# agnusmaximus/Word2Bits

Measured on AMD Instinct MI355X. Metric: training words/sec at dim=800 bitlevel=1 neg=24, higher is better.
Workload: dtype f32

## Files before the change

### word2bits_amd/csrc/w2b_device.hpp

```cpp
#pragma once
#include "w2b_internal.h"
#include <type_traits>

#ifndef W2B_T
#define W2B_T 13
#endif
#ifndef W2B_T_LOSS
#define W2B_T_LOSS W2B_T
#endif
template <bool LOSS> struct TFor { static constexpr int value = LOSS ? W2B_T_LOSS : W2B_T; };
#ifndef W2B_CA
#define W2B_CA 8
#endif
#ifndef W2B_STASH
#define W2B_STASH 8
#endif
#ifndef W2B_MINWAVES
#define W2B_MINWAVES 4
#endif

namespace {

struct QParam { int bitlevel; int steps_i; float steps_f; };

template <int QM>
__device__ __forceinline__ float quant(float x, const QParam &q) {
  if (QM == 0) return x;
  if (QM == 2) {
    const float lvl = (__builtin_fabsf(x) <= .5f) ? .25f : .75f;
    return (x < 0.f) ? -lvl : lvl;
  }
  const float sgn = (x < 0.f) ? -1.f : 1.f;
  if (QM == 1) return sgn / 3.f;
  const float mag = x * sgn;
  float lvl = 0.f;
  if (q.bitlevel >= 4) {
    int k = (int)(mag * q.steps_f + .5f);
    k = k > q.steps_i ? q.steps_i : k;
    lvl = (float)k / q.steps_f;
  }
  return sgn * lvl;
}
__device__ __forceinline__ QParam make_qparam(const W2bParams &P) {
  QParam qp;
  qp.bitlevel = P.bitlevel;
  qp.steps_i = (P.bitlevel >= 4) ? (1 << (P.bitlevel - 1)) : 1;
  qp.steps_f = (float)qp.steps_i;
  return qp;
}

template <int VEC> struct Col { float e[VEC]; };

#define W2B_MM_EXACT 4
#define W2B_EXACT_COLS 256
#ifndef W2B_XCD_STORE_AUX
#define W2B_XCD_STORE_AUX 2
#endif
template <int MM> struct Aux {
  static constexpr int load = (MM == 0 || MM == W2B_MM_EXACT) ? 16 : ((MM == 2 || MM == 5 || MM == 6) ? 2 : 0);
  static constexpr int store = (MM == 1) ? 0 : ((MM == 5) ? 2 : ((MM == 6) ? W2B_XCD_STORE_AUX : 16));
};
typedef unsigned int u32x4 __attribute__((ext_vector_type(4)));
typedef unsigned int u32x2 __attribute__((ext_vector_type(2)));
template <int VEC, int MM, int TB = -1>
__device__ __forceinline__ Col<VEC> load_col(const float *tab, long long row, int dim, int col0, unsigned tab_bytes) {
  Col<VEC> c;
  const int urow = __builtin_amdgcn_readfirstlane((int)row);
  __amdgpu_buffer_rsrc_t r;
  int soff;
  if (TB == 0 || (TB < 0 && tab_bytes)) {
    r = __builtin_amdgcn_make_buffer_rsrc((void *)tab, 0, (int)tab_bytes, 0x27000);
    soff = urow * dim * 4;
  } else {
    r = __builtin_amdgcn_make_buffer_rsrc((void *)(tab + urow * (long long)dim), 0, dim * 4, 0x27000);
    soff = 0;
  }
  if (VEC == 4) {
    u32x4 t = __builtin_amdgcn_raw_buffer_load_b128(r, col0 * 4, soff, Aux<MM>::load);
    c.e[0] = __uint_as_float(t.x); c.e[1 % VEC] = __uint_as_float(t.y);
    c.e[2 % VEC] = __uint_as_float(t.z); c.e[3 % VEC] = __uint_as_float(t.w);
  } else if (VEC == 2) {
    u32x2 t = __builtin_amdgcn_raw_buffer_load_b64(r, col0 * 4, soff, Aux<MM>::load);
    c.e[0] = __uint_as_float(t.x); c.e[1 % VEC] = __uint_as_float(t.y);
  } else {
    c.e[0] = __uint_as_float(__builtin_amdgcn_raw_buffer_load_b32(r, col0 * 4, soff, Aux<MM>::load));
  }
  return c;
}
template <int VEC, int MM, int TB = -1>
__device__ __forceinline__ void store_col(float *tab, long long row, int dim, int col0, const Col<VEC> &c,
                                          unsigned tab_bytes) {
  const int urow = __builtin_amdgcn_readfirstlane((int)row);
  __amdgpu_buffer_rsrc_t r;
  int soff;
  if (TB == 0 || (TB < 0 && tab_bytes)) {
    r = __builtin_amdgcn_make_buffer_rsrc((void *)tab, 0, (int)tab_bytes, 0x27000);
    soff = urow * dim * 4;
  } else {
    r = __builtin_amdgcn_make_buffer_rsrc((void *)(tab + urow * (long long)dim), 0, dim * 4, 0x27000);
    soff = 0;
  }
  if (VEC == 4) {
    u32x4 t;
    t.x = __float_as_uint(c.e[0]); t.y = __float_as_uint(c.e[1 % VEC]);
    t.z = __float_as_uint(c.e[2 % VEC]); t.w = __float_as_uint(c.e[3 % VEC]);
    __builtin_amdgcn_raw_buffer_store_b128(t, r, col0 * 4, soff, Aux<MM>::store);
  } else if (VEC == 2) {
    u32x2 t;
    t.x = __float_as_uint(c.e[0]); t.y = __float_as_uint(c.e[1 % VEC]);
    __builtin_amdgcn_raw_buffer_store_b64(t, r, col0 * 4, soff, Aux<MM>::store);
  } else {
    __builtin_amdgcn_raw_buffer_store_b32(__float_as_uint(c.e[0]), r, col0 * 4, soff, Aux<MM>::store);
  }
}

template <int CTRL, int ROW_MASK>
__device__ __forceinline__ float dpp_f(float x) {
  return __int_as_float(__builtin_amdgcn_update_dpp(0, __float_as_int(x), CTRL, ROW_MASK, 0xf, false));
}
template <int CTRL, int ROW_MASK>
__device__ __forceinline__ unsigned dpp_u(unsigned x) {
  return (unsigned)__builtin_amdgcn_update_dpp(0, (int)x, CTRL, ROW_MASK, 0xf, false);
}
#define W2B_DPP_QUAD_1032 0xB1
#define W2B_DPP_QUAD_2301 0x4E
#define W2B_DPP_ROW_HALF_MIRROR 0x141
#define W2B_DPP_ROW_MIRROR 0x140
#define W2B_DPP_ROW_BCAST15 0x142
#define W2B_DPP_ROW_BCAST31 0x143
__device__ __forceinline__ float wave_sum(float x) {
  x += dpp_f<W2B_DPP_QUAD_1032, 0xf>(x);
  x += dpp_f<W2B_DPP_QUAD_2301, 0xf>(x);
  x += dpp_f<W2B_DPP_ROW_HALF_MIRROR, 0xf>(x);
  x += dpp_f<W2B_DPP_ROW_MIRROR, 0xf>(x);
  x += dpp_f<W2B_DPP_ROW_BCAST15, 0xa>(x);
  x += dpp_f<W2B_DPP_ROW_BCAST31, 0xc>(x);
  return __int_as_float(__builtin_amdgcn_readlane(__float_as_int(x), 63));
}
__device__ __forceinline__ unsigned wave_xor(unsigned x) {
  x ^= dpp_u<W2B_DPP_QUAD_1032, 0xf>(x);
  x ^= dpp_u<W2B_DPP_QUAD_2301, 0xf>(x);
  x ^= dpp_u<W2B_DPP_ROW_HALF_MIRROR, 0xf>(x);
  x ^= dpp_u<W2B_DPP_ROW_MIRROR, 0xf>(x);
  x ^= dpp_u<W2B_DPP_ROW_BCAST15, 0xa>(x);
  x ^= dpp_u<W2B_DPP_ROW_BCAST31, 0xc>(x);
  return (unsigned)__builtin_amdgcn_readlane((int)x, 63);
}
__device__ __forceinline__ double wave_sum_d(double x) {
#pragma unroll
  for (int o = 32; o > 0; o >>= 1) x += __shfl_xor(x, o, 64);
  return x;
}
#define W2B_WAVE_SYNC() do { __builtin_amdgcn_fence(__ATOMIC_RELEASE, "wavefront"); __builtin_amdgcn_wave_barrier(); __builtin_amdgcn_fence(__ATOMIC_ACQUIRE, "wavefront"); } while (0)
__device__ __forceinline__ unsigned long long lane_lt_mask(int lane) {
  return lane == 0 ? 0ull : (~0ull >> (64 - lane));
}

#define W2B_LDS __attribute__((address_space(3)))
typedef float f32x4_t __attribute__((ext_vector_type(4)));
__device__ __forceinline__ Col<4> lds_ld(const W2B_LDS float *p) {
  const f32x4_t t = *(const W2B_LDS f32x4_t *)p;
  Col<4> c;
  c.e[0] = t.x; c.e[1] = t.y; c.e[2] = t.z; c.e[3] = t.w;
  return c;
}
__device__ __forceinline__ void lds_st(W2B_LDS float *p, const Col<4> &c) {
  f32x4_t t;
  t.x = c.e[0]; t.y = c.e[1]; t.z = c.e[2]; t.w = c.e[3];
  *(W2B_LDS f32x4_t *)p = t;
}

#ifdef W2B_PHASE_TIMERS
#define W2B_TICK(k) do { if (timing_) { const unsigned long long n_ = __builtin_readcyclecounter(); \
    atomicAdd(&P.shared->dbg[k], n_ - tick_); tick_ = n_; } } while (0)
#define W2B_COUNT(k) do { if (timing_) atomicAdd(&P.shared->dbg[k], 1ull); } while (0)
#else
#define W2B_TICK(k) do { } while (0)
#define W2B_COUNT(k) do { } while (0)
#endif

struct WordLds {
  int *ctx;
  int *umult;
  int *tgt;
  int *prev;
  int *cend;
  float *red;
  float *stash;
  float *xprod;
};

__device__ __forceinline__ int round4(int x) { return (x + 3) & ~3; }

__device__ __forceinline__ WordLds carve_word_lds(int *base, int window, int negative, int vec) {
  const int maxc = round4(2 * window + 1), maxt = round4(negative + 1);
  WordLds L;
  L.stash = reinterpret_cast<float *>(base);
  base += W2B_STASH * blockDim.x * vec;
  L.red = reinterpret_cast<float *>(base);
  int *p = base + 2 * W2B_T * W2B_MAXW;
  L.ctx = p; p += maxc;
  L.umult = p; p += maxc;
  L.tgt = p; p += maxt;
  L.prev = p; p += maxt;
  L.cend = p; p += maxt;
  L.xprod = nullptr;
  return L;
}


template <int T, typename IP>
__device__ __forceinline__ int prep_lists(IP tgt, IP prev, IP cend, int nt, IP ctx, IP umult, int cw,
                                          int lane) {
  W2B_WAVE_SYNC();
  for (int i0 = 0; i0 < nt; i0 += 64) {
    const int i = i0 + lane;
    const int me = (i < nt) ? tgt[i] : -1;
    int pd = -1;
    for (int j = 0; j < min(nt, i0 + 64); j++) {
      const int tj = (j >= i0) ? __builtin_amdgcn_readlane(me, j - i0) : tgt[j];
      pd = (j < i && tj == me) ? j : pd;
    }
    if (i < nt) prev[i] = pd;
  }
  if (umult) {
    for (int i0 = 0; i0 < cw; i0 += 64) {
      const int i = i0 + lane;
      const int me = (i < cw) ? ctx[i] : -1;
      bool first = true;
      int mult = 0;
      for (int j = 0; j < cw; j++) {
        const int cj = (j >= i0 && j < i0 + 64) ? __builtin_amdgcn_readlane(me, j - i0) : ctx[j];
        first = first && !(j < i && cj == me);
        mult += (j >= i && cj == me) ? 1 : 0;
      }
      if (i < cw) umult[i] = first ? mult : 0;
    }
  }
  W2B_WAVE_SYNC();
  int start = 0, k = 0;
  while (start < nt) {
    const int lim = min(start + T, nt);
    int end = lim;
    for (int i0 = start + 1; i0 < lim; i0 += 64) {
      const int i = i0 + lane;
      const bool hit = (i < lim) && (prev[i] >= start);
      const unsigned long long m = __ballot(hit);
      if (m) { end = i0 + __ffsll((long long)m) - 1; break; }
    }
    if (lane == 0) cend[k] = end;
    k++;
    start = end;
  }
  return k;
}

template <int VEC, int TB = -1>
__device__ __forceinline__ void add_col(float *tab, long long row, int dim, int col0, const Col<VEC> &d, unsigned tab_bytes) {
  const int urow = __builtin_amdgcn_readfirstlane((int)row);
  __amdgpu_buffer_rsrc_t r;
  int soff;
  if (TB == 0 || (TB < 0 && tab_bytes)) {
    r = __builtin_amdgcn_make_buffer_rsrc((void *)tab, 0, (int)tab_bytes, 0x27000);
    soff = urow * dim * 4;
  } else {
    r = __builtin_amdgcn_make_buffer_rsrc((void *)(tab + urow * (long long)dim), 0, dim * 4, 0x27000);
    soff = 0;
  }
#pragma unroll
  for (int e = 0; e < VEC; e++) (void)__builtin_amdgcn_raw_ptr_buffer_atomic_fadd_f32(d.e[e], r, (col0 + e) * 4, soff, 16);
}

template <int TB = -1>
__device__ __forceinline__ void add_col_contig(float *tab, long long row, int dim, const Col<4> &d, unsigned tab_bytes) {
  const int lane = threadIdx.x & 63, wave = threadIdx.x >> 6;
  const int urow = __builtin_amdgcn_readfirstlane((int)row);
  __amdgpu_buffer_rsrc_t r;
  int soff;
  if (TB == 0 || (TB < 0 && tab_bytes)) {
    r = __builtin_amdgcn_make_buffer_rsrc((void *)tab, 0, (int)tab_bytes, 0x27000);
    soff = urow * dim * 4;
  } else {
    r = __builtin_amdgcn_make_buffer_rsrc((void *)(tab + urow * (long long)dim), 0, dim * 4, 0x27000);
    soff = 0;
  }
  const int sel = lane & 3;
#pragma unroll
  for (int e = 0; e < 4; e++) {
    const int src = (16 * e + (lane >> 2)) << 2;
    const float p0 = __int_as_float(__builtin_amdgcn_ds_bpermute(src, __float_as_int(d.e[0])));
    const float p1 = __int_as_float(__builtin_amdgcn_ds_bpermute(src, __float_as_int(d.e[1])));
    const float p2 = __int_as_float(__builtin_amdgcn_ds_bpermute(src, __float_as_int(d.e[2])));
    const float p3 = __int_as_float(__builtin_amdgcn_ds_bpermute(src, __float_as_int(d.e[3])));
    const float v = sel == 0 ? p0 : (sel == 1 ? p1 : (sel == 2 ? p2 : p3));
    const int c = wave * 256 + e * 64 + lane;
    if (c < dim) (void)__builtin_amdgcn_raw_ptr_buffer_atomic_fadd_f32(v, r, c * 4, soff, 16);
  }
}

#define W2B_MM_XCD 5
#define W2B_MM_XHOT_ST 6
struct XHot {
  float *cu, *cv, *eu, *ev;
  unsigned *lu, *lv;
  int nu, nv;
};
__device__ __forceinline__ XHot xhot_here(const W2bParams &P) {
  XHot X;
  X.nu = P.xhot ? P.xhot_u : 0;
  X.nv = P.xhot ? P.xhot_v : 0;
  const int xcd = __builtin_amdgcn_s_getreg(20 | (0 << 6) | (3 << 11)) & (W2B_NXCD - 1);
  const long long rows = X.nu + X.nv;
  float *base = P.xhot + (long long)xcd * (2 * rows * P.dim + rows * W2B_MAXW);
  X.cu = base;
  X.cv = base + (long long)X.nu * P.dim;
  X.eu = X.cv + (long long)X.nv * P.dim;
  X.ev = X.eu + (long long)X.nu * P.dim;
  X.lu = reinterpret_cast<unsigned *>(X.ev + (long long)X.nv * P.dim);
  X.lv = X.lu + (long long)X.nu * W2B_MAXW;
  return X;
}
__device__ __forceinline__ Col<4> xhot_ld(const float *rows, int k, int n, int dim, int col0) {
  return load_col<4, W2B_MM_XCD, 0>(rows, k, dim, col0, (unsigned)(n * dim * 4));
}
__device__ __forceinline__ void xhot_st(float *rows, int k, int n, int dim, int col0, const Col<4> &c) {
  store_col<4, W2B_MM_XHOT_ST, 0>(rows, k, dim, col0, c, (unsigned)(n * dim * 4));
}
template <int MM, int TB>
__device__ __forceinline__ void xhot_merge_row(float *tab, float *copy, float *entry, unsigned *locks, int k, int n, int dim,
                                               int col0, bool active, int wave, int lane, unsigned tab_bytes, float w) {
  unsigned *lock = locks + k * W2B_MAXW + wave;
  unsigned got = 1u;
  if (lane == 0) got = __hip_atomic_exchange(lock, 1u, __ATOMIC_RELAXED, __HIP_MEMORY_SCOPE_AGENT);
  if (__builtin_amdgcn_readfirstlane((int)got) != 0) return;
  Col<4> c, e, m, o;
#pragma unroll
  for (int i = 0; i < 4; i++) { c.e[i] = 0.f; e.e[i] = 0.f; m.e[i] = 0.f; }
  if (active) {
    c = xhot_ld(copy, k, n, dim, col0);
    e = xhot_ld(entry, k, n, dim, col0);
    m = load_col<4, MM, TB>(tab, k + 1, dim, col0, tab_bytes);
  }
  bool own = false, oth = false;
#pragma unroll
  for (int i = 0; i < 4; i++) {
    own = own || __float_as_uint(c.e[i]) != __float_as_uint(e.e[i]);
    oth = oth || __float_as_uint(m.e[i]) != __float_as_uint(e.e[i]);
  }
  const bool any_own = __ballot(own) != 0ull, any_oth = __ballot(oth) != 0ull;
#pragma unroll
  for (int i = 0; i < 4; i++) o.e[i] = !any_oth ? c.e[i] : (!any_own ? m.e[i] : m.e[i] + w * (c.e[i] - m.e[i]));
  if (active) {
    if (any_own) store_col<4, MM, TB>(tab, k + 1, dim, col0, o, tab_bytes);
    if (any_oth) xhot_st(copy, k, n, dim, col0, o);
    if (any_own || any_oth) xhot_st(entry, k, n, dim, col0, o);
  }
  __builtin_amdgcn_s_waitcnt(0);
  if (lane == 0) __hip_atomic_store(lock, 0u, __ATOMIC_RELAXED, __HIP_MEMORY_SCOPE_AGENT);
}
template <int MM, int TB = -1>
__device__ __forceinline__ void xhot_merge_event(const W2bParams &P, const XHot &X, int &cursor, int col0, bool active) {
  const int lane = threadIdx.x & 63, wave = threadIdx.x >> 6;
  for (int j = 0; j < P.xhot_m; j++) {
    const int i = cursor + j;
    if (X.nu > 0 && j < X.nu)
      xhot_merge_row<MM, TB>(P.u, X.cu, X.eu, X.lu, i % X.nu, X.nu, P.dim, col0, active, wave, lane, P.tab_bytes, P.xhot_w);
    if (X.nv > 0 && j < X.nv)
      xhot_merge_row<MM, TB>(P.v, X.cv, X.ev, X.lv, i % X.nv, X.nv, P.dim, col0, active, wave, lane, P.tab_bytes, P.xhot_w);
  }
  cursor += P.xhot_m;
}

template <typename TP>
__device__ __forceinline__ float grad_scalar(const float f, const bool centre, const float alpha, TP exp_table) {
  const float label = centre ? 1.f : 0.f;
  float g;
  if (f > 6.f) g = (label - 1.f) * alpha;
  else if (f < -6.f) g = label * alpha;
  else g = (label - exp_table[(int)((f + 6.f) * 83.f)]) * alpha;
  return g;
}
__device__ __forceinline__ float log_sigmoid_term(const float f, const bool centre) {
  const float dp = centre ? f : -f;
  float sg;
  if (dp > 6.f) sg = 1.f;
  else if (dp < -6.f) sg = 1e-9f;
  else sg = 1.f / (1.f + expf(-dp));
  return logf(sg);
}

template <int QM, int VEC, bool LOSS, int MM, int ATOM = 0, int TB = -1, bool LEAN = false>
__device__ __forceinline__ void process_word(const W2bParams &P, const WordLds &L, const QParam &qp,
                                             const int cw, const int nt, const float alpha,
                                             double &loss_acc, const XHot &X) {
  static_assert(!LEAN || (VEC == 4 && MM == 0 && ATOM == 0 && TB == 0 && QM <= 2), "lean form: see w2b_workers_lean");
  constexpr bool REG = !LEAN;
  constexpr bool ATOM_U = !(VEC == 4 && ATOM < 1), ATOM_V = !(VEC == 4 && ATOM < 2);
  constexpr bool THIRDS = LEAN && QM == 1;
  constexpr float third = 1.f / 3.f;
  const int tid = threadIdx.x, lane = tid & 63, wave = tid >> 6, nwaves = blockDim.x >> 6;
  const int dim = P.dim, col0 = tid * VEC;
  const bool active = col0 < dim;
  const float ar2 = REG ? (2.f * alpha) * P.reg : 0.f;
  constexpr int TC = TFor<LOSS>::value;

  Col<VEC> x[TC];
  int rows[TC];
  int start = 0, chunk = 0, end = L.cend[0];
  auto chunk_rows = [&]() {
    const int mine = L.tgt[min(start + lane, nt - 1)];
#pragma unroll
    for (int i = 0; i < TC; i++) rows[i] = __builtin_amdgcn_readlane(mine, i);
  };
  chunk_rows();
  const int nhu = (VEC == 4) ? X.nu : 0, nhv = (VEC == 4) ? X.nv : 0;
  auto ld_u = [&](int row) -> Col<VEC> {
    if constexpr (VEC == 4) { if ((unsigned)(row - 1) < (unsigned)nhu) return xhot_ld(X.cu, row - 1, nhu, dim, col0); }
    return load_col<VEC, MM, TB>(P.u, row, dim, col0, P.tab_bytes);
  };
  [[maybe_unused]] const int atomic_rank = ATOM_V ? P.atomic_rank : 0, atomic_rank_u = ATOM_U ? P.atomic_rank_u : 0;
  auto up_u = [&](int row, const Col<VEC> &val, const Col<VEC> &d) {
    if constexpr (VEC == 4) { if ((unsigned)(row - 1) < (unsigned)nhu) { xhot_st(X.cu, row - 1, nhu, dim, col0, val); return; } }
    if constexpr (ATOM_U) { if (row <= atomic_rank_u) { add_col<VEC, TB>(P.u, row, dim, col0, d, P.tab_bytes); return; } }
    store_col<VEC, MM, TB>(P.u, row, dim, col0, val, P.tab_bytes);
  };
  auto ld_v = [&](int row) -> Col<VEC> {
    if constexpr (VEC == 4) { if ((unsigned)(row - 1) < (unsigned)nhv) return xhot_ld(X.cv, row - 1, nhv, dim, col0); }
    return load_col<VEC, MM, TB>(P.v, row, dim, col0, P.tab_bytes);
  };
  auto up_v = [&](int row, const Col<VEC> &val, const Col<VEC> &d) {
    if constexpr (VEC == 4) { if ((unsigned)(row - 1) < (unsigned)nhv) { xhot_st(X.cv, row - 1, nhv, dim, col0, val); return; } }
    if constexpr (ATOM_V) { if (row <= atomic_rank) { add_col<VEC, TB>(P.v, row, dim, col0, d, P.tab_bytes); return; } }
    store_col<VEC, MM, TB>(P.v, row, dim, col0, val, P.tab_bytes);
  };
  auto load_targets = [&](bool zero) {
#pragma unroll
    for (int i = 0; i < TC; i++) {
      if (zero) {
#pragma unroll
        for (int e = 0; e < VEC; e++) x[i].e[e] = 0.f;
      }
      if (active && start + i < end) x[i] = ld_v(rows[i]);
    }
  };
  load_targets(true);

  Col<VEC> avg;
  float regsq = 0.f;
  const bool reg_on = REG && P.reg != 0.f;
  float *fsave = reinterpret_cast<float *>(L.prev);
#pragma unroll
  for (int e = 0; e < VEC; e++) avg.e[e] = 0.f;
  for (int j0 = 0; j0 < cw; j0 += W2B_CA) {
    Col<VEC> r[W2B_CA];
#pragma unroll
    for (int jj = 0; jj < W2B_CA; jj++)
      if (active && j0 + jj < cw) r[jj] = ld_u(__builtin_amdgcn_readfirstlane(L.ctx[j0 + jj]));
#pragma unroll
    for (int jj = 0; jj < W2B_CA; jj++)
      if (active && j0 + jj < cw) {
        if (j0 + jj < W2B_STASH) {
#pragma unroll
          for (int e = 0; e < VEC; e++) L.stash[((j0 + jj) * blockDim.x + tid) * VEC + e] = r[jj].e[e];
        }
#pragma unroll
        for (int e = 0; e < VEC; e++) {
          const float q = quant<QM>(r[jj].e[e], qp);
          avg.e[e] += q;
          if (LOSS && reg_on) regsq += q * q;
        }
      }
  }
  {
    const float cwf = (float)cw;
#pragma unroll
    for (int e = 0; e < VEC; e++) avg.e[e] = active ? avg.e[e] / cwf : 0.f;
  }
  [[maybe_unused]] Col<VEC> avg3;
  if constexpr (THIRDS) {
#pragma unroll
    for (int e = 0; e < VEC; e++) avg3.e[e] = avg.e[e] * third;
  }

  Col<VEC> err;
#pragma unroll
  for (int e = 0; e < VEC; e++) err.e[e] = 0.f;
  int par = 0;
  for (;;) {
    const int n = end - start;
    float p[TC];
#pragma unroll
    for (int i = 0; i < TC; i++) {
      float t[VEC];
#pragma unroll
      for (int e = 0; e < VEC; e++) {
        if constexpr (THIRDS) t[e] = (x[i].e[e] < 0.f) ? -avg3.e[e] : avg3.e[e];
        else {
          const float q = quant<QM>(x[i].e[e], qp);
          t[e] = avg.e[e] * q;
        }
      }
      const float s = (VEC == 4) ? (t[0] + t[1 % VEC]) + (t[2 % VEC] + t[3 % VEC]) : ((VEC == 2) ? t[0] + t[1 % VEC] : t[0]);
      p[i] = active ? s : 0.f;
    }
    float *red = L.red + par * (TC * W2B_MAXW);
    if (MM == W2B_MM_EXACT) {
      float fchain = 0.f;
      for (int b0 = 0; b0 < dim; b0 += W2B_EXACT_COLS) {
        if (active && col0 >= b0 && col0 < b0 + W2B_EXACT_COLS) {
#pragma unroll
          for (int i = 0; i < TC; i++)
            if (i < n) {
#pragma unroll
              for (int e = 0; e < VEC; e++)
                L.xprod[i * (W2B_EXACT_COLS + 1) + (col0 - b0) + e] = avg.e[e] * quant<QM>(x[i].e[e], qp);
            }
        }
        __syncthreads();
        if (wave == 0 && lane < n) {
          const int cnt = min(W2B_EXACT_COLS, dim - b0);
          const float *src = L.xprod + lane * (W2B_EXACT_COLS + 1);
          for (int c = 0; c < cnt; c++) fchain += src[c];
        }
        __syncthreads();
      }
      if (wave == 0 && lane < n) {
        red[lane * W2B_MAXW] = fchain;
        for (int w = 1; w < nwaves; w++) red[lane * W2B_MAXW + w] = 0.f;
      }
    } else {
#pragma unroll
      for (int i = 0; i < TC; i++) p[i] = wave_sum(p[i]);
      if (lane == 0) {
#pragma unroll
        for (int i = 0; i < TC; i++)
          if (i < n) red[i * W2B_MAXW + wave] = p[i];
      }
    }
    __syncthreads();
    float gl = 0.f;
    if (lane < n) {
      float f = 0.f;
      for (int w = 0; w < nwaves; w++) f += red[lane * W2B_MAXW + w];
      gl = grad_scalar(f, start + lane == 0, alpha, P.exp_table);
      if (LOSS && wave == 0) fsave[start + lane] = f;
    }
#pragma unroll
    for (int i = 0; i < TC; i++) {
      if (i < n) {
        const float g = __int_as_float(__builtin_amdgcn_readlane(__float_as_int(gl), i));
        [[maybe_unused]] const float g3 = g * third;
        const bool by_add = (VEC == 4 && ATOM >= 2) && rows[i] <= atomic_rank && !((unsigned)(rows[i] - 1) < (unsigned)nhv);
        Col<VEC> dl;
        if constexpr (VEC == 4 && ATOM >= 2) {
#pragma unroll
          for (int e = 0; e < VEC; e++) dl.e[e] = 0.f;
        }
        if (active) {
#pragma unroll
          for (int e = 0; e < VEC; e++) {
            float xv = x[i].e[e];
            if (QM != 0) asm volatile("" : "+v"(xv));
            if constexpr (THIRDS) err.e[e] += (xv < 0.f) ? -g3 : g3;
            else {
              const float q = quant<QM>(xv, qp);
              if (LOSS && reg_on) regsq += q * q;
              err.e[e] += g * q;
            }
            if constexpr (REG) dl.e[e] = g * avg.e[e] - ar2 * xv;
            else dl.e[e] = g * avg.e[e] + 0.f;
            x[i].e[e] = xv + dl.e[e];
          }
          if (!by_add) up_v(rows[i], x[i], dl);
        }
        if constexpr (VEC == 4 && ATOM >= 2) {
          if (by_add) add_col_contig<TB>(P.v, rows[i], dim, dl, P.tab_bytes);
        }
      }
    }
    start = end;
    if (start >= nt) break;
    end = L.cend[++chunk];
    par ^= 1;
    chunk_rows();
    load_targets(false);
  }

  for (int j0 = 0; j0 < cw; j0 += W2B_CA) {
    Col<VEC> r[W2B_CA];
#pragma unroll
    for (int jj = 0; jj < W2B_CA; jj++)
      if (active && j0 + jj < cw && L.umult[j0 + jj] > 0) {
        const int crow = __builtin_amdgcn_readfirstlane(L.ctx[j0 + jj]);
        if (j0 + jj < W2B_STASH && crow > P.fresh_rank_u) {
#pragma unroll
          for (int e = 0; e < VEC; e++) r[jj].e[e] = L.stash[((j0 + jj) * blockDim.x + tid) * VEC + e];
        } else {
          r[jj] = ld_u(crow);
        }
      }
#pragma unroll
    for (int jj = 0; jj < W2B_CA; jj++) {
      if constexpr (VEC == 4 && ATOM >= 1) {
        if (j0 + jj < cw) {
          const int m = L.umult[j0 + jj];
          if (m > 0) {
            const int crow = __builtin_amdgcn_readfirstlane(L.ctx[j0 + jj]);
            const bool by_add = crow <= atomic_rank_u && !((unsigned)(crow - 1) < (unsigned)nhu);
            Col<VEC> dl;
#pragma unroll
            for (int e = 0; e < VEC; e++) dl.e[e] = 0.f;
            for (int k = 0; k < m; k++) {
              if (active) {
#pragma unroll
                for (int e = 0; e < VEC; e++) {
                  dl.e[e] = err.e[e] - ar2 * r[jj].e[e];
                  r[jj].e[e] = r[jj].e[e] + dl.e[e];
                }
              }
              if (by_add) add_col_contig<TB>(P.u, crow, dim, dl, P.tab_bytes);
            }
            if (!by_add && active) up_u(crow, r[jj], dl);
          }
        }
      } else {
        if (active && j0 + jj < cw) {
          const int m = L.umult[j0 + jj];
          if (m > 0) {
            const int crow = __builtin_amdgcn_readfirstlane(L.ctx[j0 + jj]);
            [[maybe_unused]] const bool by_add = ATOM_U && crow <= atomic_rank_u && !(VEC == 4 && (unsigned)(crow - 1) < (unsigned)nhu);
            Col<VEC> dl;
            for (int k = 0; k < m; k++) {
#pragma unroll
              for (int e = 0; e < VEC; e++) {
                if constexpr (REG) dl.e[e] = err.e[e] - ar2 * r[jj].e[e];
                else dl.e[e] = err.e[e];
                r[jj].e[e] = r[jj].e[e] + dl.e[e];
              }
              if constexpr (ATOM_U) { if (by_add && k + 1 < m) up_u(crow, r[jj], dl); }
            }
            up_u(crow, r[jj], dl);
          }
        }
      }
    }
  }
  if (LOSS) {
    if (wave == 0) {
      for (int j = lane; j < nt; j += 64) loss_acc += (double)log_sigmoid_term(fsave[j], j == 0);
    }
    if (reg_on) {
      const float s = wave_sum(active ? regsq : 0.f);
      if (lane == 0) loss_acc -= (double)(P.reg * s);
    }
  }
  __syncthreads();
}


template <int QM, bool LOSS, int MM>
__device__ __forceinline__ void process_word_wide(const W2bParams &P, const WordLds &L, const QParam &qp, const int cw,
                                                  const int nt, const float alpha, double &loss_acc) {
  const int tid = threadIdx.x, lane = tid & 63, wave = tid >> 6, nwaves = blockDim.x >> 6, nthr = blockDim.x;
  const int dim = P.dim;
  const float ar2 = (2.f * alpha) * P.reg;
  float *avg = P.wide_scratch + (long long)blockIdx.x * 2 * dim, *errv = avg + dim;
  auto ld = [&](float *tab, int row, int c) -> float { return load_col<1, MM>(tab, row, dim, c, P.tab_bytes).e[0]; };
  auto st = [&](float *tab, int row, int c, float x) { Col<1> v; v.e[0] = x; store_col<1, MM>(tab, row, dim, c, v, P.tab_bytes); };
  float regsq = 0.f;
  for (int c = tid; c < dim; c += nthr) {
    float s = 0.f;
    for (int j = 0; j < cw; j++) {
      const float q = quant<QM>(ld(P.u, L.ctx[j], c), qp);
      s += q;
      if (LOSS) regsq += q * q;
    }
    avg[c] = s / (float)cw;
    errv[c] = 0.f;
  }
  if (LOSS && P.reg != 0.f) {
    const float s = wave_sum(regsq);
    if (lane == 0) loss_acc -= (double)(P.reg * s);
  }
  __syncthreads();
  for (int t = 0; t < nt; t++) {
    const int row = L.tgt[t];
    float f = 0.f;
    if (MM == W2B_MM_EXACT) {
      for (int b0 = 0; b0 < dim; b0 += W2B_EXACT_COLS) {
        if (tid < W2B_EXACT_COLS && b0 + tid < dim) L.xprod[tid] = avg[b0 + tid] * quant<QM>(ld(P.v, row, b0 + tid), qp);
        __syncthreads();
        if (tid == 0) {
          const int cnt = min(W2B_EXACT_COLS, dim - b0);
          for (int c = 0; c < cnt; c++) f += L.xprod[c];
        }
        __syncthreads();
      }
      if (tid == 0) L.red[0] = f;
    } else {
      float p = 0.f;
      for (int c = tid; c < dim; c += nthr) p += avg[c] * quant<QM>(ld(P.v, row, c), qp);
      p = wave_sum(p);
      if (lane == 0) L.red[wave] = p;
      __syncthreads();
      if (tid == 0) {
        for (int w = 0; w < nwaves; w++) f += L.red[w];
        L.red[0] = f;
      }
    }
    __syncthreads();
    f = L.red[0];
    const float g = grad_scalar(f, t == 0, alpha, P.exp_table);
    if (LOSS && tid == 0) loss_acc += (double)log_sigmoid_term(f, t == 0);
    float s2 = 0.f;
    for (int c = tid; c < dim; c += nthr) {
      const float xv = ld(P.v, row, c), q = quant<QM>(xv, qp);
      if (LOSS) s2 += q * q;
      errv[c] += g * q;
      st(P.v, row, c, xv + (g * avg[c] - ar2 * xv));
    }
    if (LOSS && P.reg != 0.f) {
      s2 = wave_sum(s2);
      if (lane == 0) loss_acc -= (double)(P.reg * s2);
    }
    __syncthreads();
  }
  for (int c = tid; c < dim; c += nthr) {
    const float e = errv[c];
    for (int j = 0; j < cw; j++) {
      const int row = L.ctx[j];
      const float r = ld(P.u, row, c);
      st(P.u, row, c, r + (e - ar2 * r));
    }
  }
  __syncthreads();
}

__device__ __forceinline__ unsigned long long fast_mod(unsigned long long n, unsigned long long d,
                                                     unsigned long long magic) {
  if (d <= 1) return 0;
  const unsigned long long q = __umul64hi(n, magic);
  unsigned long long r = n - q * d;
  if (r >= d) r -= d;
  if (r >= d) r -= d;
  return r;
}
__device__ __forceinline__ long long w2b_global_progress(const W2bParams &P, long long wca_local) {
  const long long others_per_self = P.total_threads / P.num_threads - 1;
  return wca_local + (long long)P.shared->wca_others + others_per_self * (wca_local - (long long)P.shared->wca_at_sync);
}
__device__ __forceinline__ unsigned long long lcg_jump(const W2bParams &P, unsigned long long x, int k) {
  return P.jump_a[k] * x + P.jump_c[k];
}

__device__ __forceinline__ void read_sentence(const W2bParams &P, int *s_sen, unsigned long long &rng,
                                              long long &cursor, long long &wc, int &ovr, int &eof,
                                              int &len_out, const int lane) {
  int len = 0;
  bool stop = false;
  const bool sub = (P.sample > 0.f);
  if (ovr != -2) {
    const int w = ovr;
    ovr = -2;
    if (w != -1) {
      wc++;
      if (w == 0) stop = true;
      else {
        bool kept = true;
        if (sub) {
          rng = rng * W2B_LCG_A + W2B_LCG_C;
          kept = !(P.keep[w] < (float)(rng & 0xFFFF) / 65536.f);
        }
        if (kept) { if (lane == 0) s_sen[0] = w; len = 1; }
      }
    }
  }
  while (!stop) {
    const long long i = cursor + lane;
    const bool in = i < P.n_tokens;
    const int tok = in ? P.corpus[i] : 0;
    const bool isw = in && tok != 0;
    const unsigned long long mw = __ballot(isw);
    const unsigned long long lt = lane_lt_mask(lane);
    bool kept = isw;
    if (sub && isw) {
      const unsigned long long x = lcg_jump(P, rng, __popcll(mw & lt) + 1);
      kept = !(P.keep[tok] < (float)(x & 0xFFFF) / 65536.f);
    }
    const unsigned long long mk = __ballot(kept);
    const int kpos = __popcll(mk & lt);
    const bool lim = kept && (len + kpos + 1 >= W2B_MAX_SEN);
    const unsigned long long mt = __ballot(!in || (in && tok == 0) || lim);
    const unsigned long long min_ = __ballot(in);
    const int e = mt ? (__ffsll((long long)mt) - 1) : 64;
    const int ncons = e + ((e < 64 && ((min_ >> e) & 1ull)) ? 1 : 0);
    const unsigned long long cmask = (ncons >= 64) ? ~0ull : ((1ull << ncons) - 1ull);
    if (kept && lane < ncons) s_sen[len + kpos] = tok;
    len += __popcll(mk & cmask);
    wc += ncons;
    cursor += ncons;
    if (sub) rng = lcg_jump(P, rng, __popcll(mw & cmask));
    if (e < 64) {
      stop = true;
      if (!((min_ >> e) & 1ull)) {
        eof = 1;
        if (P.corpus_more && lane == 0) P.shared->corpus_overrun = 1;
      }
    }
  }
  len_out = len;
}


struct WorkerLds {
  unsigned long long rng;
  long long cursor, wc, last_wc;
  int sen_len, sen_pos, override_, eof, done, cw, nt, pad;
  float alpha;
};


template <typename DP, typename SP, typename NT>
__device__ __forceinline__ void copy_sentence(DP dst, SP src, const int len, const int t, const NT nthr) {
  for (int i = t; i < len; i += nthr) dst[i] = src[i];
}
template <typename SP>
__device__ __forceinline__ void worker_restore(const W2bWorker *G, SP S) {
  S->rng = G->rng; S->cursor = G->cursor; S->wc = G->word_count; S->last_wc = G->last_word_count;
  S->sen_len = G->sen_len; S->sen_pos = G->sen_pos; S->override_ = G->first_override;
  S->eof = 0; S->done = 0; S->cw = 0; S->nt = 0; S->alpha = 0.f;
}
template <typename SP>
__device__ __forceinline__ void worker_save(const W2bParams &P, W2bWorker *G, SP S) {
  G->rng = S->rng; G->cursor = S->cursor; G->word_count = S->wc; G->last_word_count = S->last_wc;
  G->sen_len = S->sen_len; G->sen_pos = S->sen_pos; G->first_override = S->override_;
  if (S->done) { G->done = 1; atomicAdd(&P.shared->workers_done, 1); }
}

__device__ __forceinline__ bool alpha_schedule_step(const W2bParams &P, const long long wc, long long &last_wc, const int lane,
                                                    float *stored = nullptr) {
  const bool due = wc - last_wc > 10000;
  if (due) {
    float a = 0.f;
    if (lane == 0) {
      const unsigned long long d = (unsigned long long)(wc - last_wc);
      const unsigned long long wca = atomicAdd(&P.shared->word_count_actual, d) + d;
      const long long wca_all = w2b_global_progress(P, (long long)wca);
      a = P.starting_alpha * (1.f - (float)wca_all / (float)(P.iter * P.train_words + 1));
      if ((double)a < (double)P.starting_alpha * 0.0001) a = (float)((double)P.starting_alpha * 0.0001);
      __hip_atomic_store(&P.shared->alpha, a, __ATOMIC_RELAXED, __HIP_MEMORY_SCOPE_AGENT);
    }
    if (stored) *stored = __int_as_float(__builtin_amdgcn_readfirstlane(__float_as_int(a)));
    last_wc = wc;
  }
  return due;
}

__device__ __forceinline__ void epoch_end(const W2bParams &P, const long long wc, long long &last_wc, const int lane) {
  if (lane == 0) atomicAdd(&P.shared->word_count_actual, (unsigned long long)(wc - last_wc));
  last_wc = wc;
}

__device__ __forceinline__ int window_draw(const W2bParams &P, unsigned long long &rng) {
  rng = rng * W2B_LCG_A + W2B_LCG_C;
  return (int)fast_mod(rng, (unsigned long long)P.window, P.window_magic);
}
__device__ __forceinline__ void next_position(int &sen_pos, int &sen_len) {
  sen_pos++;
  if (sen_pos >= sen_len) sen_len = 0;
}

__device__ __forceinline__ int table_entry(const W2bParams &P, const unsigned long long x) {
  return P.table[fast_mod(x >> 16, (unsigned long long)P.table_size, P.table_magic)];
}
template <bool ONE_TRIP, typename IP, typename JD, typename JA>
__device__ __forceinline__ int draw_targets(const W2bParams &P, IP tgt, const int word, unsigned long long &rng, JD jump_d, JA jump_all,
                                            const bool pref_ok, const int t_pref, const int lane) {
  const int K = P.negative;
  int cnt = 0;
  for (int d0 = 1; ONE_TRIP ? d0 == 1 : d0 <= K; d0 += 64) {
    const int d = d0 + lane;
    bool keep = false;
    int t = 0;
    if (d <= K) {
      const unsigned long long x = jump_d(rng, d);
      t = (pref_ok && d0 == 1) ? t_pref : table_entry(P, x);
      if (t == 0) t = (int)(x % (unsigned long long)(P.vocab_size - 1)) + 1;
      keep = (t != word);
    }
    const unsigned long long m = __ballot(keep);
    if (keep) tgt[1 + cnt + __popcll(m & lane_lt_mask(lane))] = t;
    cnt += __popcll(m);
  }
  if (lane == 0) tgt[0] = word;
  rng = jump_all(rng);
  return 1 + cnt;
}
template <typename JD>
__device__ __forceinline__ int table_prefetch(const W2bParams &P, const unsigned long long rng, JD jump_d, const int lane) {
  const unsigned long long xb = rng * W2B_LCG_A + W2B_LCG_C;
  return table_entry(P, jump_d(xb, lane + 1));
}

template <typename F>
hipError_t dispatch_q(int bitlevel, F &&f) {
#ifdef W2B_QUICK_BUILD
  return f(std::integral_constant<int, 1>());
#else
  switch (bitlevel) {
    case 0: return f(std::integral_constant<int, 0>());
    case 1: return f(std::integral_constant<int, 1>());
    case 2: return f(std::integral_constant<int, 2>());
    default: return f(std::integral_constant<int, 3>());
  }
#endif
}


template <typename F>
hipError_t dispatch_mm_exact(int mem_mode, int exact, F &&f);

template <typename F>
hipError_t dispatch_mm(int mem_mode, F &&f) {
  switch (mem_mode) {
    case 1: return f(std::integral_constant<int, 1>());
#ifdef W2B_EXPERIMENTAL_MEMMODES
    case 2: return f(std::integral_constant<int, 2>());
    case 3: return f(std::integral_constant<int, 3>());
#endif
    default: return f(std::integral_constant<int, 0>());
  }
}

template <typename F>
hipError_t dispatch_mm_exact(int mem_mode, int exact, F &&f) {
  if (exact) return f(std::integral_constant<int, W2B_MM_EXACT>());
  return dispatch_mm(mem_mode, f);
}

}
```

Baseline: 27.72 million.

## Reduce all target dot products with one transposed DPP butterfly on the lean path

Replaces the per-target full-wave DPP reduction, which ran TC separate six-step reductions and then a readlane, with a transposed recursive-halving reduction. At each DPP level every lane keeps one half and sends the other, so all TC partial sums (up to 16) finish in a single butterfly tree. A permlane16/32 swap stage then completes the cross-row sum, and lanes in the first row write their target's total into shared memory. This cuts the number of cross-lane ops and VALU adds per negative-sample batch. The cost is a more complex lane-to-slot mapping, masking and select logic, and it only applies when LEAN is set. It also depends on permlane swap builtins, which the code assumes the target supports.

```diff
diff --git a/word2bits_amd/csrc/w2b_device.hpp b/word2bits_amd/csrc/w2b_device.hpp
--- a/word2bits_amd/csrc/w2b_device.hpp
+++ b/word2bits_amd/csrc/w2b_device.hpp
@@ -136,6 +136,55 @@
   x += dpp_f<W2B_DPP_ROW_BCAST15, 0xa>(x);
   x += dpp_f<W2B_DPP_ROW_BCAST31, 0xc>(x);
   return __int_as_float(__builtin_amdgcn_readlane(__float_as_int(x), 63));
+}
+constexpr int tsum_slot(int j) { return j ^ (((j >> 2) & 1) * 3) ^ (((j >> 3) & 1) * 4); }
+constexpr bool tsum_slot_ok() {
+  unsigned seen = 0;
+  for (int j = 0; j < 16; j++) {
+    const int s = tsum_slot(j);
+    if (s < 0 || s > 15) return false;
+    seen |= 1u << s;
+    if (tsum_slot(j ^ 1) != (s ^ 1)) return false;
+    if (tsum_slot(j ^ 2) != (s ^ 2)) return false;
+    if (tsum_slot((j & 8) | (7 - (j & 7))) != (s ^ 4)) return false;
+    if (tsum_slot(15 - j) != (s ^ 8)) return false;
+  }
+  return seen == 0xffffu;
+}
+static_assert(tsum_slot_ok(), "tsum_slot: every DPP partner must hold the other half of the same target");
+template <int K> __device__ __forceinline__ float tsum_dpp(float x) {
+  static_assert(K >= 0 && K < 4, "levels inside a row of 16");
+  if constexpr (K == 0) return dpp_f<W2B_DPP_QUAD_1032, 0xf>(x);
+  else if constexpr (K == 1) return dpp_f<W2B_DPP_QUAD_2301, 0xf>(x);
+  else if constexpr (K == 2) return dpp_f<W2B_DPP_ROW_HALF_MIRROR, 0xf>(x);
+  else return dpp_f<W2B_DPP_ROW_MIRROR, 0xf>(x);
+}
+template <int LVL, int BASE, int TC, class F>
+__device__ __forceinline__ float tsum_level(const int slot, F &&part) {
+  if constexpr (LVL == 0) return part(BASE);
+  else {
+    constexpr int K = LVL - 1;
+    const float a = tsum_level<K, BASE, TC>(slot, part);
+    if constexpr (BASE + (1 << K) < TC) {
+      const float b = tsum_level<K, BASE + (1 << K), TC>(slot, part);
+      unsigned m = (unsigned)-((slot >> K) & 1);
+      asm("" : "+v"(m));
+      const unsigned ua = __float_as_uint(a), ub = __float_as_uint(b);
+      const float keep = __uint_as_float((ub & m) | (ua & ~m)), give = __uint_as_float((ua & m) | (ub & ~m));
+      return keep + tsum_dpp<K>(give);
+    } else {
+      return a + tsum_dpp<K>(a);
+    }
+  }
+}
+template <int TC, class F>
+__device__ __forceinline__ float wave_sum_transposed(const int slot, F &&part) {
+  static_assert(TC >= 1 && TC <= 16, "one target per lane of a row");
+  float x = tsum_level<4, 0, TC>(slot, part);
+  const auto r16 = __builtin_amdgcn_permlane16_swap(__float_as_uint(x), __float_as_uint(x), false, false);
+  x = __uint_as_float(r16[0]) + __uint_as_float(r16[1]);
+  const auto r32 = __builtin_amdgcn_permlane32_swap(__float_as_uint(x), __float_as_uint(x), false, false);
+  return __uint_as_float(r32[0]) + __uint_as_float(r32[1]);
 }
 __device__ __forceinline__ unsigned wave_xor(unsigned x) {
   x ^= dpp_u<W2B_DPP_QUAD_1032, 0xf>(x);
@@ -486,11 +535,12 @@
 #pragma unroll
   for (int e = 0; e < VEC; e++) err.e[e] = 0.f;
   int par = 0;
+  [[maybe_unused]] int l = lane;
+  if constexpr (LEAN) asm volatile("" : "+v"(l));
+  [[maybe_unused]] const int slot = (l & 15) ^ (((l >> 2) & 1) * 3) ^ (((l >> 3) & 1) * 4);
   for (;;) {
     const int n = end - start;
-    float p[TC];
-#pragma unroll
-    for (int i = 0; i < TC; i++) {
+    auto part = [&](const int i) -> float {
       float t[VEC];
 #pragma unroll
       for (int e = 0; e < VEC; e++) {
@@ -501,8 +551,9 @@
         }
       }
       const float s = (VEC == 4) ? (t[0] + t[1 % VEC]) + (t[2 % VEC] + t[3 % VEC]) : ((VEC == 2) ? t[0] + t[1 % VEC] : t[0]);
-      p[i] = active ? s : 0.f;
-    }
+      if constexpr (THIRDS) return s;
+      else return active ? s : 0.f;
+    };
     float *red = L.red + par * (TC * W2B_MAXW);
     if (MM == W2B_MM_EXACT) {
       float fchain = 0.f;
@@ -528,7 +579,13 @@
         red[lane * W2B_MAXW] = fchain;
         for (int w = 1; w < nwaves; w++) red[lane * W2B_MAXW + w] = 0.f;
       }
+    } else if constexpr (LEAN) {
+      const float tot = wave_sum_transposed<TC>(slot, part);
+      if (l < 16 && slot < n) red[slot * W2B_MAXW + wave] = tot;
     } else {
+      float p[TC];
+#pragma unroll
+      for (int i = 0; i < TC; i++) p[i] = part(i);
 #pragma unroll
       for (int i = 0; i < TC; i++) p[i] = wave_sum(p[i]);
       if (lane == 0) {
```

Result: faster. 28.10 million (median of 6 runs) (+1.4%).
